# rafaelghiorzi/YOLO-MS

Measured on AMD Instinct MI355X. Metric: images/sec (train+infer) YOLO-MS-S 640x640 bf16 at 1/2/4/8 MI355X; mAP parity, higher is better.
Workload: dtype bf16; 1 GPU; configs[2]: YOLO-MS-S (reference YOLOv8-'s' graph) 640x640 bf16 training, B=64/GPU, fwd+loss+bwd+SGD-nesterov step; global_batch=64, per_gpu_batch=64, img=640, parallelism=dp1, hip_graph=False

## Files before the change

yolo-ms_amd/csrc/stem.hip:

```cpp
#include <algorithm>
#include <cstdlib>

#include "conv_common.hpp"

namespace yms {

constexpr int ST_TH = 8, ST_TW = 32;
constexpr int ST_IH = 2 * ST_TH + 1;
constexpr int ST_IW = 2 * ST_TW + 4;
constexpr int ST_IN = 3 * ST_IH * ST_IW;

struct StemParams {
  const float* x;
  const float* w;
  char* y;
  int y_ld, y_off;
  const float* scale;
  const float* shift;
  int act;
  float* stats;
  int stats_ld;
  float* stats_cnt;
  int N, CI, H, W, CO, Ho, Wo, tiles_x, tiles_y;
  int vec4;
  int ysplit, tps;
};

template <typename T>
__device__ __forceinline__ uint32_t pack2(float a, float b) {
  const T ta = (T)a, tb = (T)b;
  return (uint32_t)__builtin_bit_cast(uint16_t, ta) | ((uint32_t)__builtin_bit_cast(uint16_t, tb) << 16);
}

template <typename T, int NT, bool STATS>
__global__ __launch_bounds__(256) void conv_stem_kernel(StemParams p) {
  constexpr int CP = NT * 32;
  constexpr int OP = CP * (int)sizeof(T) + 16;
  constexpr int OUT_B = 4 * 64 * OP;
  constexpr int IN_B = ST_IN * 4;
  constexpr int RED_B = 4 * 3 * CP * 4;
  __shared__ __attribute__((aligned(16))) char smem[IN_B + OUT_B + RED_B];
  float* xin = reinterpret_cast<float*>(smem);
  float* red = reinterpret_cast<float*>(smem + IN_B + OUT_B);

  const int per_col = p.tiles_x * p.ysplit;
  const int n = blockIdx.x / per_col, rem = blockIdx.x - n * per_col;
  const int tx = rem % p.tiles_x, ty0 = (rem / p.tiles_x) * p.tps, ty1 = min(p.tiles_y, ty0 + p.tps);
  const int ox0 = tx * ST_TW;
  const int tid = threadIdx.x, lane = tid & 63, wave = tid >> 6;
  const int lr = lane & 31, lh = lane >> 5;
  const float* xn = p.x + (long)n * p.CI * p.H * p.W;
  const int ix0 = 2 * ox0;

  constexpr int NV = 3 * ST_IH * 16, NVI = (NV + 255) / 256;
  f32x4 v[NVI];
  float hcol = 0.f;
  auto load_tile = [&](int ty) {
    const int iy0 = 2 * ty * ST_TH - 1;
#pragma unroll
    for (int j = 0; j < NVI; ++j) {
      const int it = tid + 256 * j;
      const int row = it >> 4, q = it & 15;
      const int ci = row / ST_IH, iy = iy0 + row - ci * ST_IH, ix = ix0 + 4 * q;
      v[j] = f32x4{0.f, 0.f, 0.f, 0.f};
      if (it < NV && ci < p.CI && iy >= 0 && iy < p.H) {
        const float* src = xn + ((long)ci * p.H + iy) * p.W + ix;
        if (p.vec4) {
          if (ix < p.W) v[j] = *reinterpret_cast<const f32x4*>(src);
        } else {
#pragma unroll
          for (int e = 0; e < 4; ++e) v[j][e] = ix + e < p.W ? src[e] : 0.f;
        }
      }
    }
    if (tid < 3 * ST_IH) {
      const int ci = tid / ST_IH, iy = iy0 + tid - ci * ST_IH;
      hcol = (ci < p.CI && iy >= 0 && iy < p.H && ix0 >= 1) ? xn[((long)ci * p.H + iy) * p.W + ix0 - 1] : 0.f;
    }
  };

  const int K = p.CI * 9;
  u32x4 bfr[NT][2];
#pragma unroll
  for (int b = 0; b < NT; ++b) {
    const int co = 32 * b + lr;
#pragma unroll
    for (int s = 0; s < 2; ++s) {
      float wv[8];
#pragma unroll
      for (int j = 0; j < 8; ++j) {
        const int k = 16 * s + 8 * lh + j;
        wv[j] = (co < p.CO && k < K) ? p.w[(long)co * K + k] : 0.0f;
      }
      bfr[b][s] = u32x4{pack2<T>(wv[0], wv[1]), pack2<T>(wv[2], wv[3]), pack2<T>(wv[4], wv[5]),
                        pack2<T>(wv[6], wv[7])};
    }
  }
  int koff[2][8];
#pragma unroll
  for (int s = 0; s < 2; ++s)
#pragma unroll
    for (int j = 0; j < 8; ++j) {
      const int k = 16 * s + 8 * lh + j;
      const int ci = k / 9, t = k - ci * 9, kh = t / 3, kw = t - kh * 3;
      koff[s][j] = k < K ? (ci * ST_IH + kh) * ST_IW + kw + 3 : -1;
    }
  float sc[NT], sh[NT];
#pragma unroll
  for (int b = 0; b < NT; ++b) {
    const int co = 32 * b + lr;
    sc[b] = (!STATS && co < p.CO && p.scale) ? p.scale[co] : 1.0f;
    sh[b] = (!STATS && co < p.CO && p.shift) ? p.shift[co] : 0.0f;
  }
  auto prow = [&](int i) { return (i & 3) + 8 * (i >> 2) + 4 * lh; };
  const int vx = min(ST_TW, p.Wo - ox0);
  const int cch = p.CO / 8;
  T* y = reinterpret_cast<T*>(p.y);
  char* ot = smem + IN_B + wave * 64 * OP;

  load_tile(ty0);
  for (int ty = ty0; ty < ty1; ++ty) {
    const int oy0 = ty * ST_TH;
#pragma unroll
    for (int j = 0; j < NVI; ++j) {
      const int it = tid + 256 * j;
      if (it < NV) *reinterpret_cast<f32x4*>(xin + (it >> 4) * ST_IW + 4 + 4 * (it & 15)) = v[j];
    }
    if (tid < 3 * ST_IH) xin[tid * ST_IW + 3] = hcol;
    __syncthreads();
    if (ty + 1 < ty1) load_tile(ty + 1);
    f32x16 acc[2][NT];
#pragma unroll
    for (int a = 0; a < 2; ++a) {
#pragma unroll
      for (int b = 0; b < NT; ++b)
#pragma unroll
        for (int i = 0; i < 16; ++i) acc[a][b][i] = 0.0f;
      const int base = 2 * (2 * wave + a) * ST_IW + 2 * lr;
#pragma unroll
      for (int s = 0; s < 2; ++s) {
        float av[8];
#pragma unroll
        for (int j = 0; j < 8; ++j) av[j] = koff[s][j] >= 0 ? xin[base + koff[s][j]] : 0.0f;
        const u32x4 af = u32x4{pack2<T>(av[0], av[1]), pack2<T>(av[2], av[3]), pack2<T>(av[4], av[5]),
                               pack2<T>(av[6], av[7])};
#pragma unroll
        for (int b = 0; b < NT; ++b) acc[a][b] = Mfma<T>::mma(af, bfr[b][s], acc[a][b]);
      }
    }
    bool rowok[2];
#pragma unroll
    for (int a = 0; a < 2; ++a) rowok[a] = oy0 + 2 * wave + a < p.Ho;
    if constexpr (STATS) {
#pragma unroll
      for (int b = 0; b < NT; ++b) {
        float s = 0.f, cntv = 0.f;
#pragma unroll
        for (int a = 0; a < 2; ++a)
#pragma unroll
          for (int i = 0; i < 16; ++i)
            if (rowok[a] && prow(i) < vx) { s += acc[a][b][i]; cntv += 1.f; }
        s += __shfl_xor(s, 32);
        cntv += __shfl_xor(cntv, 32);
        const float mu = cntv > 0.f ? s / cntv : 0.f;
        float q = 0.f;
#pragma unroll
        for (int a = 0; a < 2; ++a)
#pragma unroll
          for (int i = 0; i < 16; ++i)
            if (rowok[a] && prow(i) < vx) {
              const float d = acc[a][b][i] - mu;
              q += d * d;
            }
        q += __shfl_xor(q, 32);
        if (lh == 0) {
          red[(wave * 3 + 0) * CP + 32 * b + lr] = cntv;
          red[(wave * 3 + 1) * CP + 32 * b + lr] = s;
          red[(wave * 3 + 2) * CP + 32 * b + lr] = q;
        }
      }
    }
#pragma unroll
    for (int b = 0; b < NT; ++b) {
      const int co = 32 * b + lr;
#pragma unroll
      for (int a = 0; a < 2; ++a)
#pragma unroll
        for (int i = 0; i < 16; ++i) {
          float val = acc[a][b][i];
          if (!STATS) {
            val = val * sc[b] + sh[b];
            if (p.act == YMS_ACT_SILU) val = silu_f(val);
          }
          *reinterpret_cast<T*>(ot + (a * 32 + prow(i)) * OP + co * (int)sizeof(T)) = (T)val;
        }
    }
    __syncthreads();
    if constexpr (STATS) {
      const int tile = (n * p.tiles_y + ty) * p.tiles_x + tx;
      if (tid < p.CO) {
        float nt = 0.f, st = 0.f;
#pragma unroll
        for (int w = 0; w < 4; ++w) { nt += red[(w * 3 + 0) * CP + tid]; st += red[(w * 3 + 1) * CP + tid]; }
        const float mean = nt > 0.f ? st / nt : 0.f;
        float m2 = 0.f;
#pragma unroll
        for (int w = 0; w < 4; ++w) {
          const float nw = red[(w * 3 + 0) * CP + tid];
          if (nw > 0.f) {
            const float d = red[(w * 3 + 1) * CP + tid] / nw - mean;
            m2 += red[(w * 3 + 2) * CP + tid] + nw * d * d;
          }
        }
        float* so = p.stats + (long)tile * 2 * p.stats_ld;
        so[tid] = st;
        so[p.stats_ld + tid] = m2;
        if (tid == 0) p.stats_cnt[tile] = nt;
      }
    }
    for (int it = lane; it < 64 * cch; it += 64) {
      const int px = it / cch, ch = it - px * cch;
      const int a = px >> 5, ox = ox0 + (px & 31), oy = oy0 + 2 * wave + a;
      if (oy < p.Ho && ox < p.Wo) {
        const u32x4 val = *reinterpret_cast<const u32x4*>(ot + px * OP + ch * 16);
        *reinterpret_cast<u32x4*>(y + (((long)n * p.Ho + oy) * p.Wo + ox) * p.y_ld + p.y_off + 8 * ch) = val;
      }
    }
  }
}

template <typename T, int NT>
__global__ __launch_bounds__(256) void conv_stem_wgrad_kernel(StemParams p, const T* gy, int gy_ld, int gy_off,
                                                              const T* z, int z_ld, int z_off, const float* mi,
                                                              const float* coef, float* ws) {
  constexpr int CP = NT * 32;
  constexpr int DP = 256 + 8;
  constexpr int IN_B = ST_IN * 4;
  constexpr int DZ_B = CP * DP * (int)sizeof(T);
  constexpr int RED_B = 4 * CP * 32 * 4;
  constexpr int MAIN_B = (IN_B + DZ_B) > RED_B ? (IN_B + DZ_B) : RED_B;
  __shared__ __attribute__((aligned(16))) char smem[MAIN_B + 4 * CP * 4];
  float* xin = reinterpret_cast<float*>(smem);
  T* dzt = reinterpret_cast<T*>(smem + IN_B);
  float* red = reinterpret_cast<float*>(smem);
  float (*prm)[CP] = reinterpret_cast<float (*)[CP]>(smem + MAIN_B);

  const int per_col = p.tiles_x * p.ysplit;
  const int n = blockIdx.x / per_col, rem = blockIdx.x - n * per_col;
  const int tx = rem % p.tiles_x, ty0 = (rem / p.tiles_x) * p.tps, ty1 = min(p.tiles_y, ty0 + p.tps);
  const int ox0 = tx * ST_TW;
  const int tid = threadIdx.x, lane = tid & 63, wave = tid >> 6;
  const int lr = lane & 31, lh = lane >> 5;
  const float* xn = p.x + (long)n * p.CI * p.H * p.W;
  const int ix0 = 2 * ox0, K = p.CI * 9, cch = p.CO / 8;

  constexpr int NPAIR = 128 * CP / 8, NDZ = (NPAIR + 255) / 256;
  for (int c = tid; c < CP; c += 256) {
    float sc = 0.f, sh = 0.f, a0 = 0.f, bz = 0.f;
    if (c < p.CO) {
      sc = p.scale[c];
      sh = p.shift[c];
      const float mu = mi[c], is = mi[p.CO + c];
      bz = -sc * coef[p.CO + c] * is;
      a0 = -sc * coef[c] - bz * mu;
    }
    prm[0][c] = sc; prm[1][c] = sh; prm[2][c] = a0; prm[3][c] = bz;
  }
  f32x16 acc[NT];
#pragma unroll
  for (int b = 0; b < NT; ++b)
#pragma unroll
    for (int i = 0; i < 16; ++i) acc[b][i] = 0.0f;
  const int kk = lr;
  const int kci = kk / 9, kt = kk - kci * 9, kkh = kt / 3, kkw = kt - kkh * 3;
  const bool kok = kk < K;

  constexpr int NV = 3 * ST_IH * 16, NVI = (NV + 255) / 256;
  f32x4 xv[NVI];
  float hcol = 0.f;
  Raw8<T> graw[NDZ][2], zraw[NDZ][2];
  auto load_tile = [&](int ty) {
    const int oy0 = ty * ST_TH, iy0 = 2 * oy0 - 1;
#pragma unroll
    for (int j = 0; j < NVI; ++j) {
      const int it = tid + 256 * j;
      const int row = it >> 4, q = it & 15;
      const int ci = row / ST_IH, iy = iy0 + row - ci * ST_IH, ix = ix0 + 4 * q;
      xv[j] = f32x4{0.f, 0.f, 0.f, 0.f};
      if (it < NV && ci < p.CI && iy >= 0 && iy < p.H) {
        const float* src = xn + ((long)ci * p.H + iy) * p.W + ix;
        if (p.vec4) {
          if (ix < p.W) xv[j] = *reinterpret_cast<const f32x4*>(src);
        } else {
#pragma unroll
          for (int e = 0; e < 4; ++e) xv[j][e] = ix + e < p.W ? src[e] : 0.f;
        }
      }
    }
    if (tid < 3 * ST_IH) {
      const int ci = tid / ST_IH, iy = iy0 + tid - ci * ST_IH;
      hcol = (ci < p.CI && iy >= 0 && iy < p.H && ix0 >= 1) ? xn[((long)ci * p.H + iy) * p.W + ix0 - 1] : 0.f;
    }
#pragma unroll
    for (int j = 0; j < NDZ; ++j) {
      const int it = tid + 256 * j;
      const int pp = it / (CP / 8), g = it - pp * (CP / 8);
      const int oy = oy0 + (pp >> 4), c0 = 8 * g;
#pragma unroll
      for (int h = 0; h < 2; ++h) {
        const int ox = ox0 + 2 * (pp & 15) + h;
#pragma unroll
        for (int k = 0; k < (int)(sizeof(T) / 2); ++k) { graw[j][h].v[k] = u32x4{0u, 0u, 0u, 0u}; zraw[j][h].v[k] = graw[j][h].v[k]; }
        if (it < NPAIR && g < cch && oy < p.Ho && ox < p.Wo) {
          const long pix = ((long)n * p.Ho + oy) * p.Wo + ox;
          load_raw8(gy + pix * gy_ld + gy_off + c0, 8, graw[j][h]);
          load_raw8(z + pix * z_ld + z_off + c0, 8, zraw[j][h]);
        }
      }
    }
  };

  load_tile(ty0);
  for (int ty = ty0; ty < ty1; ++ty) {
    __syncthreads();
#pragma unroll
    for (int j = 0; j < NVI; ++j) {
      const int it = tid + 256 * j;
      if (it < NV) *reinterpret_cast<f32x4*>(xin + (it >> 4) * ST_IW + 4 + 4 * (it & 15)) = xv[j];
    }
    if (tid < 3 * ST_IH) xin[tid * ST_IW + 3] = hcol;
#pragma unroll
    for (int j = 0; j < NDZ; ++j) {
      const int it = tid + 256 * j;
      if (it < NPAIR) {
        const int pp = it / (CP / 8), g = it - pp * (CP / 8), c0 = 8 * g;
        const int oy = ty * ST_TH + (pp >> 4);
        float o[2][8];
#pragma unroll
        for (int h = 0; h < 2; ++h) {
          const bool valid = g < cch && oy < p.Ho && ox0 + 2 * (pp & 15) + h < p.Wo;
          float gv[8], zv[8];
          unpack8(graw[j][h], gv);
          unpack8(zraw[j][h], zv);
#pragma unroll
          for (int e = 0; e < 8; ++e) {
            const int c = c0 + e;
            const float sc = prm[0][c], sh = prm[1][c], a0 = prm[2][c], bz = prm[3][c];
            float da = gv[e];
            if (p.act == YMS_ACT_SILU) da *= dsilu_f(zv[e] * sc + sh);
            o[h][e] = valid ? sc * da + a0 + bz * zv[e] : 0.f;
          }
        }
#pragma unroll
        for (int e = 0; e < 8; ++e)
          *reinterpret_cast<uint32_t*>(dzt + (c0 + e) * DP + 2 * pp) = pack2<T>(o[0][e], o[1][e]);
      }
    }
    __syncthreads();
    if (ty + 1 < ty1) load_tile(ty + 1);
#pragma unroll
    for (int a = 0; a < 2; ++a) {
      const int prow = 2 * wave + a;
#pragma unroll
      for (int s2 = 0; s2 < 2; ++s2) {
        const int p0 = 16 * s2 + 8 * lh;
        float bv[8];
        const int base = (kci * ST_IH + 2 * prow + kkh) * ST_IW + kkw + 3 + 2 * p0;
#pragma unroll
        for (int j = 0; j < 8; ++j) bv[j] = kok ? xin[base + 2 * j] : 0.f;
        const u32x4 bf = u32x4{pack2<T>(bv[0], bv[1]), pack2<T>(bv[2], bv[3]), pack2<T>(bv[4], bv[5]),
                               pack2<T>(bv[6], bv[7])};
#pragma unroll
        for (int b = 0; b < NT; ++b) {
          const u32x4 af = *reinterpret_cast<const u32x4*>(dzt + (32 * b + lr) * DP + 64 * wave + 32 * a + p0);
          acc[b] = Mfma<T>::mma(af, bf, acc[b]);
        }
      }
    }
  }
  __syncthreads();
#pragma unroll
  for (int b = 0; b < NT; ++b)
#pragma unroll
    for (int i = 0; i < 16; ++i) {
      const int co = 32 * b + (i & 3) + 8 * (i >> 2) + 4 * lh;
      red[(wave * CP + co) * 32 + lr] = acc[b][i];
    }
  __syncthreads();
  for (int it = tid; it < p.CO * K; it += 256) {
    const int co = it / K, k = it - co * K;
    const float v = ((red[(0 * CP + co) * 32 + k] + red[(1 * CP + co) * 32 + k]) + red[(2 * CP + co) * 32 + k]) +
                    red[(3 * CP + co) * 32 + k];
    ws[(long)blockIdx.x * p.CO * K + it] = v;
  }
}

__global__ __launch_bounds__(1024) void stem_wgrad_reduce_kernel(const float* ws, int blocks, int items, float* dw,
                                                                 int accumulate) {
  __shared__ float red[16][64];
  const int lane = threadIdx.x & 63, w = threadIdx.x >> 6;
  const int j = blockIdx.x * 64 + lane;
  float s0 = 0.f, s1 = 0.f, s2 = 0.f, s3 = 0.f;
  if (j < items) {
    int b = w;
    for (; b + 48 < blocks; b += 64) {
      s0 += ws[(long)b * items + j];
      s1 += ws[(long)(b + 16) * items + j];
      s2 += ws[(long)(b + 32) * items + j];
      s3 += ws[(long)(b + 48) * items + j];
    }
    for (; b < blocks; b += 16) s0 += ws[(long)b * items + j];
  }
  red[w][lane] = (s0 + s1) + (s2 + s3);
  __syncthreads();
  for (int h = 8; h >= 1; h >>= 1) {
    if (w < h) red[w][lane] += red[w + h][lane];
    __syncthreads();
  }
  if (w == 0 && j < items) dw[j] = accumulate ? dw[j] + red[0][lane] : red[0][lane];
}

static bool stem_shape_ok(const yms_conv_shape* s) {
  return s && s->n > 0 && s->h > 0 && s->w > 0 && s->cin >= 1 && s->cin <= 3 && s->cout >= 8 && s->cout % 8 == 0 &&
         s->cout <= 96 && s->k == 3 && s->stride == 2 && s->pad == 1 && s->ho == (s->h - 1) / 2 + 1 &&
         s->wo == (s->w - 1) / 2 + 1 && (s->dtype == YMS_BF16 || s->dtype == YMS_F16);
}

static int stem_tiles(const yms_conv_shape* s, int& tx, int& ty) {
  tx = (s->wo + ST_TW - 1) / ST_TW;
  ty = (s->ho + ST_TH - 1) / ST_TH;
  return s->n * tx * ty;
}

static unsigned stem_strips(const yms_conv_shape* s, StemParams& p, long target) {
  const long cols = (long)s->n * p.tiles_x;
  const int want = (int)std::max(1l, std::min<long>(p.tiles_y, (target + cols - 1) / cols));
  p.tps = (p.tiles_y + want - 1) / want;
  p.ysplit = (p.tiles_y + p.tps - 1) / p.tps;
  return (unsigned)(cols * p.ysplit);
}

constexpr long STEM_WG_BLOCKS = 1024;

}

using namespace yms;

extern "C" {

int yms_conv_stem_supported(const yms_conv_shape* s) { return stem_shape_ok(s) ? 1 : 0; }

int yms_conv_stem_stats_rows(const yms_conv_shape* s) {
  if (!stem_shape_ok(s)) return 0;
  int tx, ty;
  return stem_tiles(s, tx, ty);
}

yms_status yms_conv_stem_fwd(const yms_conv_shape* s, const float* x, const float* w, void* y, int y_ld, int y_off,
                             const float* scale, const float* shift, int act, float* stats, int stats_ld,
                             void* stream) {
  if (!s || !x || !w || !y) return YMS_ERR_INVALID;
  if (!stem_shape_ok(s)) return YMS_ERR_UNSUPPORTED;
  if (y_ld % 8 || y_off % 8 || y_off + s->cout > y_ld) return YMS_ERR_INVALID;
  if (stats && stats_ld < s->cout) return YMS_ERR_INVALID;
  if ((long)s->n * s->cin * s->h * s->w >= (1l << 31)) return YMS_ERR_UNSUPPORTED;
  StemParams p{};
  p.x = x; p.w = w; p.y = (char*)y; p.y_ld = y_ld; p.y_off = y_off;
  p.scale = scale; p.shift = shift; p.act = act;
  p.stats = stats; p.stats_ld = stats_ld;
  p.N = s->n; p.CI = s->cin; p.H = s->h; p.W = s->w; p.CO = s->cout; p.Ho = s->ho; p.Wo = s->wo;
  const int tiles = stem_tiles(s, p.tiles_x, p.tiles_y);
  p.vec4 = (s->w % 4 == 0 && ((uintptr_t)x & 15) == 0) ? 1 : 0;
  if (stats) p.stats_cnt = stats + (long)tiles * 2 * stats_ld;
  const unsigned blocks = stem_strips(s, p, 1024);
  hipStream_t st = (hipStream_t)stream;
  const int nt = (s->cout + 31) / 32;
#define YMS_STEM(TT)                                                                                         \
  do {                                                                                                       \
    if (stats) {                                                                                             \
      if (nt == 1) hipLaunchKernelGGL((conv_stem_kernel<TT, 1, true>), dim3(blocks), dim3(256), 0, st, p);    \
      else if (nt == 2) hipLaunchKernelGGL((conv_stem_kernel<TT, 2, true>), dim3(blocks), dim3(256), 0, st, p); \
      else hipLaunchKernelGGL((conv_stem_kernel<TT, 3, true>), dim3(blocks), dim3(256), 0, st, p);            \
    } else {                                                                                                 \
      if (nt == 1) hipLaunchKernelGGL((conv_stem_kernel<TT, 1, false>), dim3(blocks), dim3(256), 0, st, p);   \
      else if (nt == 2) hipLaunchKernelGGL((conv_stem_kernel<TT, 2, false>), dim3(blocks), dim3(256), 0, st, p); \
      else hipLaunchKernelGGL((conv_stem_kernel<TT, 3, false>), dim3(blocks), dim3(256), 0, st, p);           \
    }                                                                                                        \
  } while (0)
  if (s->dtype == YMS_BF16) YMS_STEM(bf16);
  else YMS_STEM(f16);
#undef YMS_STEM
  return launch_status();
}

size_t yms_conv_stem_wgrad_ws_bytes(const yms_conv_shape* s) {
  if (!stem_shape_ok(s)) return 0;
  StemParams p{};
  stem_tiles(s, p.tiles_x, p.tiles_y);
  return (size_t)stem_strips(s, p, STEM_WG_BLOCKS) * s->cout * s->cin * 9 * sizeof(float);
}

yms_status yms_conv_stem_wgrad(const yms_conv_shape* s, const float* x, const void* gy, int gy_ld, int gy_off,
                               const void* z, int z_ld, int z_off, const float* scale, const float* shift,
                               const float* mean_invstd, const float* coef, int act, float* ws, size_t ws_bytes,
                               float* dw, int accumulate, void* stream) {
  if (!s || !x || !gy || !z || !scale || !shift || !mean_invstd || !coef || !ws || !dw) return YMS_ERR_INVALID;
  if (!stem_shape_ok(s)) return YMS_ERR_UNSUPPORTED;
  if (gy_ld % 8 || gy_off % 8 || gy_off + s->cout > gy_ld || z_ld % 8 || z_off % 8 || z_off + s->cout > z_ld)
    return YMS_ERR_INVALID;
  if (ws_bytes < yms_conv_stem_wgrad_ws_bytes(s)) return YMS_ERR_INVALID;
  if ((long)s->n * s->cin * s->h * s->w >= (1l << 31)) return YMS_ERR_UNSUPPORTED;
  StemParams p{};
  p.x = x; p.scale = scale; p.shift = shift; p.act = act;
  p.N = s->n; p.CI = s->cin; p.H = s->h; p.W = s->w; p.CO = s->cout; p.Ho = s->ho; p.Wo = s->wo;
  stem_tiles(s, p.tiles_x, p.tiles_y);
  p.vec4 = (s->w % 4 == 0 && ((uintptr_t)x & 15) == 0) ? 1 : 0;
  const unsigned blocks = stem_strips(s, p, STEM_WG_BLOCKS);
  hipStream_t st = (hipStream_t)stream;
  const int nt = (s->cout + 31) / 32;
#define YMS_STEM_WG(TT)                                                                                        \
  do {                                                                                                         \
    const TT* g_ = (const TT*)gy; const TT* z_ = (const TT*)z;                                                 \
    if (nt == 1) hipLaunchKernelGGL((conv_stem_wgrad_kernel<TT, 1>), dim3(blocks), dim3(256), 0, st, p, g_, gy_ld, \
                                    gy_off, z_, z_ld, z_off, mean_invstd, coef, ws);                          \
    else if (nt == 2) hipLaunchKernelGGL((conv_stem_wgrad_kernel<TT, 2>), dim3(blocks), dim3(256), 0, st, p, g_, \
                                         gy_ld, gy_off, z_, z_ld, z_off, mean_invstd, coef, ws);              \
    else hipLaunchKernelGGL((conv_stem_wgrad_kernel<TT, 3>), dim3(blocks), dim3(256), 0, st, p, g_, gy_ld,    \
                            gy_off, z_, z_ld, z_off, mean_invstd, coef, ws);                                  \
  } while (0)
  if (s->dtype == YMS_BF16) YMS_STEM_WG(bf16);
  else YMS_STEM_WG(f16);
#undef YMS_STEM_WG
  yms_status e = launch_status();
  if (e != YMS_OK) return e;
  const int items = s->cout * s->cin * 9;
  hipLaunchKernelGGL(stem_wgrad_reduce_kernel, dim3((items + 63) / 64), dim3(1024), 0, st, ws, (int)blocks, items, dw,
                     accumulate);
  return launch_status();
}

}
```

Before: 3809 images/sec.

## Restructure stem conv prefetch with branchless loads, templated vec4 path and fast stats

Moves the input footprint loading of the stem forward and wgrad kernels into a shared helper. Loads become unconditional with masked addresses and a validity bitmask, and the vec4 choice becomes a compile-time template split. The forward kernel now writes the next tile to LDS after the output sync, adds a fast path for BatchNorm statistics on full tiles, replaces the per-lane store loop division with incremental indexing, and raises occupancy hints for NT==1. The wgrad kernel overlaps the gy/z prefetch for the next tile with the dz computation. In exchange it adds an extra barrier per tile and higher register pressure, and the compute order of the statistics changes slightly.

```diff
diff --git a/yolo-ms_amd/csrc/stem.hip b/yolo-ms_amd/csrc/stem.hip
--- a/yolo-ms_amd/csrc/stem.hip
+++ b/yolo-ms_amd/csrc/stem.hip
@@ -32,14 +32,70 @@
   return (uint32_t)__builtin_bit_cast(uint16_t, ta) | ((uint32_t)__builtin_bit_cast(uint16_t, tb) << 16);
 }
 
-template <typename T, int NT, bool STATS>
-__global__ __launch_bounds__(256) void conv_stem_kernel(StemParams p) {
-  constexpr int CP = NT * 32;
-  constexpr int OP = CP * (int)sizeof(T) + 16;
-  constexpr int OUT_B = 4 * 64 * OP;
-  constexpr int IN_B = ST_IN * 4;
-  constexpr int RED_B = 4 * 3 * CP * 4;
-  __shared__ __attribute__((aligned(16))) char smem[IN_B + OUT_B + RED_B];
+template <bool V4>
+struct StemFootprint {
+  static constexpr int NV = 3 * ST_IH * 16, NVI = (NV + 255) / 256;
+  f32x4 v[NVI];
+  float hcol;
+  unsigned okm;
+
+  __device__ __forceinline__ void load(const float* xn, int tid, int iy0, int ix0, int CI, int H, int W, bool live) {
+    okm = 0;
+#pragma unroll
+    for (int j = 0; j < NVI; ++j) {
+      const int it = tid + 256 * j;
+      const int row = it >> 4, q = it & 15;
+      const int ci = row / ST_IH, iy = iy0 + row - ci * ST_IH, ix = ix0 + 4 * q;
+      const bool rok = live && it < NV && ci < CI && iy >= 0 && iy < H;
+      const long off = ((long)ci * H + iy) * W + ix;
+      if constexpr (V4) {
+        const bool ok = rok && ix < W;
+        v[j] = *reinterpret_cast<const f32x4*>(xn + (ok ? off : 0l));
+        okm |= ok ? 0xfu << (4 * j) : 0u;
+      } else {
+        v[j] = f32x4{0.f, 0.f, 0.f, 0.f};
+        if (rok) {
+#pragma unroll
+          for (int e = 0; e < 4; ++e) v[j][e] = ix + e < W ? xn[off + e] : 0.f;
+        }
+        okm |= 0xfu << (4 * j);
+      }
+    }
+    const int ci = tid / ST_IH, iy = iy0 + tid - ci * ST_IH;
+    const bool ok = live && tid < 3 * ST_IH && ci < CI && iy >= 0 && iy < H && ix0 >= 1;
+    hcol = xn[ok ? ((long)ci * H + iy) * W + ix0 - 1 : 0l];
+    okm |= ok ? 1u << (4 * NVI) : 0u;
+  }
+  __device__ __forceinline__ void write(float* xin, int tid) const {
+#pragma unroll
+    for (int j = 0; j < NVI; ++j) {
+      const int it = tid + 256 * j;
+      f32x4 val = v[j];
+      asm volatile("" : "+v"(val));
+#pragma unroll
+      for (int e = 0; e < 4; ++e) val[e] = (okm >> (4 * j + e) & 1u) ? val[e] : 0.f;
+      if (it < NV) *reinterpret_cast<f32x4*>(xin + (it >> 4) * ST_IW + 4 + 4 * (it & 15)) = val;
+    }
+    float hv = hcol;
+    asm volatile("" : "+v"(hv));
+    if (tid < 3 * ST_IH) xin[tid * ST_IW + 3] = (okm >> (4 * NVI) & 1u) ? hv : 0.f;
+  }
+};
+
+template <typename T, int NT>
+struct StemFwdLds {
+  static constexpr int CP = NT * 32;
+  static constexpr int OP = CP * (int)sizeof(T) + 16;
+  static constexpr int OUT_B = 4 * 64 * OP;
+  static constexpr int IN_B = ST_IN * 4;
+  static constexpr int RED_B = 4 * 3 * CP * 4;
+  static constexpr int BYTES = IN_B + OUT_B + RED_B;
+};
+
+template <typename T, int NT, bool STATS, bool V4>
+__device__ __forceinline__ void conv_stem_strip(const StemParams& p, char* smem) {
+  using L = StemFwdLds<T, NT>;
+  constexpr int CP = L::CP, OP = L::OP, OUT_B = L::OUT_B, IN_B = L::IN_B;
   float* xin = reinterpret_cast<float*>(smem);
   float* red = reinterpret_cast<float*>(smem + IN_B + OUT_B);
 
@@ -52,32 +108,7 @@
   const float* xn = p.x + (long)n * p.CI * p.H * p.W;
   const int ix0 = 2 * ox0;
 
-  constexpr int NV = 3 * ST_IH * 16, NVI = (NV + 255) / 256;
-  f32x4 v[NVI];
-  float hcol = 0.f;
-  auto load_tile = [&](int ty) {
-    const int iy0 = 2 * ty * ST_TH - 1;
-#pragma unroll
-    for (int j = 0; j < NVI; ++j) {
-      const int it = tid + 256 * j;
-      const int row = it >> 4, q = it & 15;
-      const int ci = row / ST_IH, iy = iy0 + row - ci * ST_IH, ix = ix0 + 4 * q;
-      v[j] = f32x4{0.f, 0.f, 0.f, 0.f};
-      if (it < NV && ci < p.CI && iy >= 0 && iy < p.H) {
-        const float* src = xn + ((long)ci * p.H + iy) * p.W + ix;
-        if (p.vec4) {
-          if (ix < p.W) v[j] = *reinterpret_cast<const f32x4*>(src);
-        } else {
-#pragma unroll
-          for (int e = 0; e < 4; ++e) v[j][e] = ix + e < p.W ? src[e] : 0.f;
-        }
-      }
-    }
-    if (tid < 3 * ST_IH) {
-      const int ci = tid / ST_IH, iy = iy0 + tid - ci * ST_IH;
-      hcol = (ci < p.CI && iy >= 0 && iy < p.H && ix0 >= 1) ? xn[((long)ci * p.H + iy) * p.W + ix0 - 1] : 0.f;
-    }
-  };
+  StemFootprint<V4> fp;
 
   const int K = p.CI * 9;
   u32x4 bfr[NT][2];
@@ -90,20 +121,24 @@
 #pragma unroll
       for (int j = 0; j < 8; ++j) {
         const int k = 16 * s + 8 * lh + j;
-        wv[j] = (co < p.CO && k < K) ? p.w[(long)co * K + k] : 0.0f;
+        const bool ok = co < p.CO && k < K;
+        const float t = p.w[ok ? (long)co * K + k : 0l];
+        wv[j] = ok ? t : 0.0f;
       }
       bfr[b][s] = u32x4{pack2<T>(wv[0], wv[1]), pack2<T>(wv[2], wv[3]), pack2<T>(wv[4], wv[5]),
                         pack2<T>(wv[6], wv[7])};
     }
   }
   int koff[2][8];
+  unsigned kpad = 0;
 #pragma unroll
   for (int s = 0; s < 2; ++s)
 #pragma unroll
     for (int j = 0; j < 8; ++j) {
       const int k = 16 * s + 8 * lh + j;
       const int ci = k / 9, t = k - ci * 9, kh = t / 3, kw = t - kh * 3;
-      koff[s][j] = k < K ? (ci * ST_IH + kh) * ST_IW + kw + 3 : -1;
+      koff[s][j] = k < K ? (ci * ST_IH + kh) * ST_IW + kw + 3 : 0;
+      kpad |= k < K ? 0u : 1u << (8 * s + j);
     }
   float sc[NT], sh[NT];
 #pragma unroll
@@ -118,17 +153,15 @@
   T* y = reinterpret_cast<T*>(p.y);
   char* ot = smem + IN_B + wave * 64 * OP;
 
-  load_tile(ty0);
+  const int px_l = lane / cch, ch_l = lane - px_l * cch, px_d = 64 / cch, ch_d = 64 - px_d * cch;
+
+  fp.load(xn, tid, 2 * ty0 * ST_TH - 1, ix0, p.CI, p.H, p.W, true);
+  fp.write(xin, tid);
+  __syncthreads();
   for (int ty = ty0; ty < ty1; ++ty) {
     const int oy0 = ty * ST_TH;
-#pragma unroll
-    for (int j = 0; j < NVI; ++j) {
-      const int it = tid + 256 * j;
-      if (it < NV) *reinterpret_cast<f32x4*>(xin + (it >> 4) * ST_IW + 4 + 4 * (it & 15)) = v[j];
-    }
-    if (tid < 3 * ST_IH) xin[tid * ST_IW + 3] = hcol;
-    __syncthreads();
-    if (ty + 1 < ty1) load_tile(ty + 1);
+    const bool has_next = ty + 1 < ty1;
+    fp.load(xn, tid, 2 * (ty + 1) * ST_TH - 1, ix0, p.CI, p.H, p.W, has_next);
     f32x16 acc[2][NT];
 #pragma unroll
     for (int a = 0; a < 2; ++a) {
@@ -141,7 +174,10 @@
       for (int s = 0; s < 2; ++s) {
         float av[8];
 #pragma unroll
-        for (int j = 0; j < 8; ++j) av[j] = koff[s][j] >= 0 ? xin[base + koff[s][j]] : 0.0f;
+        for (int j = 0; j < 8; ++j) {
+          const float t = xin[base + koff[s][j]];
+          av[j] = (kpad >> (8 * s + j) & 1u) ? 0.0f : t;
+        }
         const u32x4 af = u32x4{pack2<T>(av[0], av[1]), pack2<T>(av[2], av[3]), pack2<T>(av[4], av[5]),
                                pack2<T>(av[6], av[7])};
 #pragma unroll
@@ -152,26 +188,44 @@
 #pragma unroll
     for (int a = 0; a < 2; ++a) rowok[a] = oy0 + 2 * wave + a < p.Ho;
     if constexpr (STATS) {
+#pragma clang fp contract(off)
+      const bool full = rowok[0] && rowok[1] && vx == ST_TW;
 #pragma unroll
       for (int b = 0; b < NT; ++b) {
-        float s = 0.f, cntv = 0.f;
-#pragma unroll
-        for (int a = 0; a < 2; ++a)
-#pragma unroll
-          for (int i = 0; i < 16; ++i)
-            if (rowok[a] && prow(i) < vx) { s += acc[a][b][i]; cntv += 1.f; }
-        s += __shfl_xor(s, 32);
-        cntv += __shfl_xor(cntv, 32);
-        const float mu = cntv > 0.f ? s / cntv : 0.f;
-        float q = 0.f;
-#pragma unroll
-        for (int a = 0; a < 2; ++a)
-#pragma unroll
-          for (int i = 0; i < 16; ++i)
-            if (rowok[a] && prow(i) < vx) {
+        float s = 0.f, cntv = 0.f, q = 0.f;
+        if (full) {
+#pragma unroll
+          for (int a = 0; a < 2; ++a)
+#pragma unroll
+            for (int i = 0; i < 16; ++i) s += acc[a][b][i];
+          s += __shfl_xor(s, 32);
+          cntv = 64.f;
+          const float mu = s / 64.f;
+#pragma unroll
+          for (int a = 0; a < 2; ++a)
+#pragma unroll
+            for (int i = 0; i < 16; ++i) {
               const float d = acc[a][b][i] - mu;
-              q += d * d;
+              q = __builtin_fmaf(d, d, q);
             }
+        } else {
+#pragma unroll
+          for (int a = 0; a < 2; ++a)
+#pragma unroll
+            for (int i = 0; i < 16; ++i)
+              if (rowok[a] && prow(i) < vx) { s += acc[a][b][i]; cntv += 1.f; }
+          s += __shfl_xor(s, 32);
+          cntv += __shfl_xor(cntv, 32);
+          const float mu = cntv > 0.f ? s / cntv : 0.f;
+#pragma unroll
+          for (int a = 0; a < 2; ++a)
+#pragma unroll
+            for (int i = 0; i < 16; ++i)
+              if (rowok[a] && prow(i) < vx) {
+                const float d = acc[a][b][i] - mu;
+                q = __builtin_fmaf(d, d, q);
+              }
+        }
         q += __shfl_xor(q, 32);
         if (lh == 0) {
           red[(wave * 3 + 0) * CP + 32 * b + lr] = cntv;
@@ -196,6 +250,7 @@
         }
     }
     __syncthreads();
+    if (has_next) fp.write(xin, tid);
     if constexpr (STATS) {
       const int tile = (n * p.tiles_y + ty) * p.tiles_x + tx;
       if (tid < p.CO) {
@@ -218,28 +273,44 @@
         if (tid == 0) p.stats_cnt[tile] = nt;
       }
     }
-    for (int it = lane; it < 64 * cch; it += 64) {
-      const int px = it / cch, ch = it - px * cch;
+    for (int r = 0, px = px_l, ch = ch_l; r < cch; ++r) {
       const int a = px >> 5, ox = ox0 + (px & 31), oy = oy0 + 2 * wave + a;
       if (oy < p.Ho && ox < p.Wo) {
         const u32x4 val = *reinterpret_cast<const u32x4*>(ot + px * OP + ch * 16);
         *reinterpret_cast<u32x4*>(y + (((long)n * p.Ho + oy) * p.Wo + ox) * p.y_ld + p.y_off + 8 * ch) = val;
       }
-    }
-  }
+      px += px_d;
+      ch += ch_d;
+      if (ch >= cch) { ch -= cch; ++px; }
+    }
+    __syncthreads();
+  }
+}
+
+template <typename T, int NT, bool STATS>
+__global__ __launch_bounds__(256, NT == 1 ? 3 : 1) void conv_stem_kernel(StemParams p) {
+  __shared__ __attribute__((aligned(16))) char smem[StemFwdLds<T, NT>::BYTES];
+  if (p.vec4) conv_stem_strip<T, NT, STATS, true>(p, smem);
+  else conv_stem_strip<T, NT, STATS, false>(p, smem);
 }
 
 template <typename T, int NT>
-__global__ __launch_bounds__(256) void conv_stem_wgrad_kernel(StemParams p, const T* gy, int gy_ld, int gy_off,
-                                                              const T* z, int z_ld, int z_off, const float* mi,
-                                                              const float* coef, float* ws) {
-  constexpr int CP = NT * 32;
-  constexpr int DP = 256 + 8;
-  constexpr int IN_B = ST_IN * 4;
-  constexpr int DZ_B = CP * DP * (int)sizeof(T);
-  constexpr int RED_B = 4 * CP * 32 * 4;
-  constexpr int MAIN_B = (IN_B + DZ_B) > RED_B ? (IN_B + DZ_B) : RED_B;
-  __shared__ __attribute__((aligned(16))) char smem[MAIN_B + 4 * CP * 4];
+struct StemWgLds {
+  static constexpr int CP = NT * 32;
+  static constexpr int DP = 256 + 8;
+  static constexpr int IN_B = ST_IN * 4;
+  static constexpr int DZ_B = CP * DP * (int)sizeof(T);
+  static constexpr int RED_B = 4 * CP * 32 * 4;
+  static constexpr int MAIN_B = (IN_B + DZ_B) > RED_B ? (IN_B + DZ_B) : RED_B;
+  static constexpr int BYTES = MAIN_B + 4 * CP * 4;
+};
+
+template <typename T, int NT, bool V4>
+__device__ __forceinline__ void conv_stem_wgrad_strip(const StemParams& p, const T* gy, int gy_ld, int gy_off,
+                                                      const T* z, int z_ld, int z_off, const float* mi,
+                                                      const float* coef, float* ws, char* smem) {
+  using L = StemWgLds<T, NT>;
+  constexpr int CP = L::CP, DP = L::DP, IN_B = L::IN_B, MAIN_B = L::MAIN_B;
   float* xin = reinterpret_cast<float*>(smem);
   T* dzt = reinterpret_cast<T*>(smem + IN_B);
   float* red = reinterpret_cast<float*>(smem);
@@ -275,89 +346,61 @@
   const int kci = kk / 9, kt = kk - kci * 9, kkh = kt / 3, kkw = kt - kkh * 3;
   const bool kok = kk < K;
 
-  constexpr int NV = 3 * ST_IH * 16, NVI = (NV + 255) / 256;
-  f32x4 xv[NVI];
-  float hcol = 0.f;
+  StemFootprint<V4> fp;
   Raw8<T> graw[NDZ][2], zraw[NDZ][2];
-  auto load_tile = [&](int ty) {
-    const int oy0 = ty * ST_TH, iy0 = 2 * oy0 - 1;
-#pragma unroll
-    for (int j = 0; j < NVI; ++j) {
-      const int it = tid + 256 * j;
-      const int row = it >> 4, q = it & 15;
-      const int ci = row / ST_IH, iy = iy0 + row - ci * ST_IH, ix = ix0 + 4 * q;
-      xv[j] = f32x4{0.f, 0.f, 0.f, 0.f};
-      if (it < NV && ci < p.CI && iy >= 0 && iy < p.H) {
-        const float* src = xn + ((long)ci * p.H + iy) * p.W + ix;
-        if (p.vec4) {
-          if (ix < p.W) xv[j] = *reinterpret_cast<const f32x4*>(src);
-        } else {
-#pragma unroll
-          for (int e = 0; e < 4; ++e) xv[j][e] = ix + e < p.W ? src[e] : 0.f;
-        }
-      }
-    }
-    if (tid < 3 * ST_IH) {
-      const int ci = tid / ST_IH, iy = iy0 + tid - ci * ST_IH;
-      hcol = (ci < p.CI && iy >= 0 && iy < p.H && ix0 >= 1) ? xn[((long)ci * p.H + iy) * p.W + ix0 - 1] : 0.f;
-    }
+  const bool silu = p.act == YMS_ACT_SILU;
+  static_assert(NPAIR % 256 == 0, "dz items must fill the block");
+  auto item_valid = [&](int ty, int j, int h) {
+    const int it = tid + 256 * j, pp = it / (CP / 8), g = it - pp * (CP / 8);
+    return g < cch && ty * ST_TH + (pp >> 4) < p.Ho && ox0 + 2 * (pp & 15) + h < p.Wo;
+  };
+  auto load_gz = [&](int ty, int j, bool live) {
+    const int it = tid + 256 * j, pp = it / (CP / 8), g = it - pp * (CP / 8);
+    const int oy = ty * ST_TH + (pp >> 4);
+#pragma unroll
+    for (int h = 0; h < 2; ++h) {
+      const bool ok = live && item_valid(ty, j, h);
+      const long pix = (long)n * p.Ho * p.Wo + (ok ? (long)oy * p.Wo + ox0 + 2 * (pp & 15) + h : 0l);
+      const int c0 = ok ? 8 * g : 0;
+      load_raw8(gy + pix * gy_ld + gy_off + c0, 8, graw[j][h]);
+      load_raw8(z + pix * z_ld + z_off + c0, 8, zraw[j][h]);
+    }
+  };
+
+  fp.load(xn, tid, 2 * ty0 * ST_TH - 1, ix0, p.CI, p.H, p.W, true);
+#pragma unroll
+  for (int j = 0; j < NDZ; ++j) load_gz(ty0, j, true);
+  for (int ty = ty0; ty < ty1; ++ty) {
+    const bool has_next = ty + 1 < ty1;
+    __syncthreads();
+    fp.write(xin, tid);
+    fp.load(xn, tid, 2 * (ty + 1) * ST_TH - 1, ix0, p.CI, p.H, p.W, has_next);
 #pragma unroll
     for (int j = 0; j < NDZ; ++j) {
       const int it = tid + 256 * j;
-      const int pp = it / (CP / 8), g = it - pp * (CP / 8);
-      const int oy = oy0 + (pp >> 4), c0 = 8 * g;
+      const int pp = it / (CP / 8), g = it - pp * (CP / 8), c0 = 8 * g;
+      float o[2][8];
 #pragma unroll
       for (int h = 0; h < 2; ++h) {
-        const int ox = ox0 + 2 * (pp & 15) + h;
-#pragma unroll
-        for (int k = 0; k < (int)(sizeof(T) / 2); ++k) { graw[j][h].v[k] = u32x4{0u, 0u, 0u, 0u}; zraw[j][h].v[k] = graw[j][h].v[k]; }
-        if (it < NPAIR && g < cch && oy < p.Ho && ox < p.Wo) {
-          const long pix = ((long)n * p.Ho + oy) * p.Wo + ox;
-          load_raw8(gy + pix * gy_ld + gy_off + c0, 8, graw[j][h]);
-          load_raw8(z + pix * z_ld + z_off + c0, 8, zraw[j][h]);
-        }
-      }
-    }
-  };
-
-  load_tile(ty0);
-  for (int ty = ty0; ty < ty1; ++ty) {
+        const bool valid = item_valid(ty, j, h);
+        float gv[8], zv[8];
+        unpack8(graw[j][h], gv);
+        unpack8(zraw[j][h], zv);
+#pragma unroll
+        for (int e = 0; e < 8; ++e) {
+          const int c = c0 + e;
+          const float sc = prm[0][c], sh = prm[1][c], a0 = prm[2][c], bz = prm[3][c];
+          const float ds = gv[e] * dsilu_f(zv[e] * sc + sh);
+          const float da = silu ? ds : gv[e];
+          o[h][e] = valid ? sc * da + a0 + bz * zv[e] : 0.f;
+        }
+      }
+      load_gz(ty + 1, j, has_next);
+#pragma unroll
+      for (int e = 0; e < 8; ++e)
+        *reinterpret_cast<uint32_t*>(dzt + (c0 + e) * DP + 2 * pp) = pack2<T>(o[0][e], o[1][e]);
+    }
     __syncthreads();
-#pragma unroll
-    for (int j = 0; j < NVI; ++j) {
-      const int it = tid + 256 * j;
-      if (it < NV) *reinterpret_cast<f32x4*>(xin + (it >> 4) * ST_IW + 4 + 4 * (it & 15)) = xv[j];
-    }
-    if (tid < 3 * ST_IH) xin[tid * ST_IW + 3] = hcol;
-#pragma unroll
-    for (int j = 0; j < NDZ; ++j) {
-      const int it = tid + 256 * j;
-      if (it < NPAIR) {
-        const int pp = it / (CP / 8), g = it - pp * (CP / 8), c0 = 8 * g;
-        const int oy = ty * ST_TH + (pp >> 4);
-        float o[2][8];
-#pragma unroll
-        for (int h = 0; h < 2; ++h) {
-          const bool valid = g < cch && oy < p.Ho && ox0 + 2 * (pp & 15) + h < p.Wo;
-          float gv[8], zv[8];
-          unpack8(graw[j][h], gv);
-          unpack8(zraw[j][h], zv);
-#pragma unroll
-          for (int e = 0; e < 8; ++e) {
-            const int c = c0 + e;
-            const float sc = prm[0][c], sh = prm[1][c], a0 = prm[2][c], bz = prm[3][c];
-            float da = gv[e];
-            if (p.act == YMS_ACT_SILU) da *= dsilu_f(zv[e] * sc + sh);
-            o[h][e] = valid ? sc * da + a0 + bz * zv[e] : 0.f;
-          }
-        }
-#pragma unroll
-        for (int e = 0; e < 8; ++e)
-          *reinterpret_cast<uint32_t*>(dzt + (c0 + e) * DP + 2 * pp) = pack2<T>(o[0][e], o[1][e]);
-      }
-    }
-    __syncthreads();
-    if (ty + 1 < ty1) load_tile(ty + 1);
 #pragma unroll
     for (int a = 0; a < 2; ++a) {
       const int prow = 2 * wave + a;
@@ -365,9 +408,12 @@
       for (int s2 = 0; s2 < 2; ++s2) {
         const int p0 = 16 * s2 + 8 * lh;
         float bv[8];
-        const int base = (kci * ST_IH + 2 * prow + kkh) * ST_IW + kkw + 3 + 2 * p0;
-#pragma unroll
-        for (int j = 0; j < 8; ++j) bv[j] = kok ? xin[base + 2 * j] : 0.f;
+        const int base = kok ? (kci * ST_IH + 2 * prow + kkh) * ST_IW + kkw + 3 + 2 * p0 : 0;
+#pragma unroll
+        for (int j = 0; j < 8; ++j) {
+          const float t = xin[base + 2 * j];
+          bv[j] = kok ? t : 0.f;
+        }
         const u32x4 bf = u32x4{pack2<T>(bv[0], bv[1]), pack2<T>(bv[2], bv[3]), pack2<T>(bv[4], bv[5]),
                                pack2<T>(bv[6], bv[7])};
 #pragma unroll
@@ -393,6 +439,15 @@
                     red[(3 * CP + co) * 32 + k];
     ws[(long)blockIdx.x * p.CO * K + it] = v;
   }
+}
+
+template <typename T, int NT>
+__global__ __launch_bounds__(256) void conv_stem_wgrad_kernel(StemParams p, const T* gy, int gy_ld, int gy_off,
+                                                              const T* z, int z_ld, int z_off, const float* mi,
+                                                              const float* coef, float* ws) {
+  __shared__ __attribute__((aligned(16))) char smem[StemWgLds<T, NT>::BYTES];
+  if (p.vec4) conv_stem_wgrad_strip<T, NT, true>(p, gy, gy_ld, gy_off, z, z_ld, z_off, mi, coef, ws, smem);
+  else conv_stem_wgrad_strip<T, NT, false>(p, gy, gy_ld, gy_off, z, z_ld, z_off, mi, coef, ws, smem);
 }
 
 __global__ __launch_bounds__(1024) void stem_wgrad_reduce_kernel(const float* ws, int blocks, int items, float* dw,
```

Result: no change. 3842 images/sec (median of 6 runs) (+0.9%).
